# kazuotani14/iLQR

Measured on AMD Instinct MI355X. Metric: iLQR iterations/sec (batch x T timesteps/sec), acrobot T=500 batch=4096, higher is better.
Workload: dtype f64; 1 GPU; acrobot n=4 m=1 T=499 (500 knots), box-QP limits active, FD derivatives + backward/box-QP + 11-alpha search + accept, fixed work; batch_per_gpu=4096, global_batch=4096, T=499, parallelism=batch shards x1, one all_gather of costs

## Files before the change

ilqr_amd/csrc/backward_hex.hpp:

```cpp
#pragma once
#include "solve_tile.hpp"

namespace ilqr {

#ifndef ILQR_COMMIT_ROLLED
#define ILQR_COMMIT_ROLLED 1
#endif

constexpr int HT = 4;
#ifndef ILQR_HEX_SLOT_PAD
#define ILQR_HEX_SLOT_PAD 8
#endif
#ifndef ILQR_HEX_PAIR_PERM
#define ILQR_HEX_PAIR_PERM 1
#endif
#ifndef ILQR_HEX_CAND_T
#define ILQR_HEX_CAND_T 1
#endif
constexpr bool kHexCandT = ILQR_HEX_CAND_T != 0;

template <int NX, int NU, class real, int SLOTS_>
struct HexRing {
  static constexpr int US = Rec<NX, NU>::SIZE;
  static constexpr int PAIRS = (Rec<NX, NU>::SIZE + NU + 1) / 2;
  static constexpr int ROW = 2 * HT;
  static constexpr int PAD = ROW - 2 * TW;
  static constexpr int ELEMS = PAIRS * ROW + ILQR_HEX_SLOT_PAD;
  static constexpr int SLOTS = SLOTS_;
  static constexpr bool PERM = (ILQR_HEX_PAIR_PERM != 0) && NX == 4 && NU == 1;
  static constexpr int pos(int pair) { return PERM ? hex_pair_pos(pair) : pair; }
};

constexpr int kHexKnotsPerRound = 64 / HT;
constexpr int kHexSlots = 24;
constexpr int kHexLead = 7;
static_assert(kHexSlots > kHexLead + kHexKnotsPerRound - 1, "a round must not reach a slot the chain has not left");

template <class real, int NX, int NU>
struct HexPair {
  using RS = HexRing<NX, NU, real, kHexSlots>;
  alignas(16) real ring[RS::SLOTS * RS::ELEMS];
  int rounds_done;
  int consumer_at;
  int passes_started;
  unsigned long long pass_lanes;
};

template <class P>
struct HexGate {
  static constexpr bool kRing = true;
  P& sh;
  const int T, nrounds, N;
  int pass = -1, have = 0;
  int g_next = 0, slot_next = 0, slot_cur = 0;
  __device__ __forceinline__ HexGate(P& s, int T_) : sh(s), T(T_), nrounds((T_ + 1 + kHexKnotsPerRound - 1) / kHexKnotsPerRound), N(nrounds * kHexKnotsPerRound) {}
  __device__ __forceinline__ void begin_pass() {
    pass++;
    have = pass * N;
    g_next = pass * N;
    slot_next = g_next % P::RS::SLOTS;
    __hip_atomic_store(&sh.pass_lanes, __ballot(1), __ATOMIC_RELAXED, __HIP_MEMORY_SCOPE_WORKGROUP);
    __hip_atomic_store(&sh.passes_started, pass + 1, __ATOMIC_RELEASE, __HIP_MEMORY_SCOPE_WORKGROUP);
  }
  __device__ __forceinline__ int slot(int) const { return slot_cur; }
  __device__ __forceinline__ void wait(int) {
    const int G = g_next++;
    slot_cur = slot_next;
    slot_next = (slot_next + 1 == P::RS::SLOTS) ? 0 : slot_next + 1;
    __hip_atomic_store(&sh.consumer_at, G, __ATOMIC_RELAXED, __HIP_MEMORY_SCOPE_WORKGROUP);
    if (G < have) return;
    const int round = pass * nrounds + (G - pass * N) / kHexKnotsPerRound;
    while (__hip_atomic_load(&sh.rounds_done, __ATOMIC_ACQUIRE, __HIP_MEMORY_SCOPE_WORKGROUP) <= round) __builtin_amdgcn_s_sleep(1);
    have = pass * N + ((G - pass * N) / kHexKnotsPerRound + 1) * kHexKnotsPerRound;
  }
  __device__ __forceinline__ void finish() {
    __hip_atomic_store(&sh.consumer_at, 0x3fffffff, __ATOMIC_RELAXED, __HIP_MEMORY_SCOPE_WORKGROUP);
    __hip_atomic_store(&sh.passes_started, -1, __ATOMIC_RELEASE, __HIP_MEMORY_SCOPE_WORKGROUP);
  }
};

__device__ __forceinline__ int hex_first(unsigned long long bal, int t4) {
  return __builtin_ctzll(((bal >> t4) & 0x000F000F000F000Full) | 0x8000000000000000ull);
}
__device__ __forceinline__ void qp1_search_hex(QP1StateT<double>& q, int j, int t4, double step_j0, const double* __restrict__ lds_steps) {
  const double t_x1 = clamp_of(q.x + step_j0 * q.search, q.lo, q.hi);
  const double t_v1 = qp1_value(q, t_x1);
  const bool t_pass = !qp1_armijo_fails(q, t_v1, step_j0);
  const int pp = hex_first(__ballot(t_pass), t4);
  const bool success = pp < 52;
  const int jw = success ? (((pp >> 4) << 2) | (pp & 3)) : 0;
#ifdef ILQR_EXP_NO_STEP_LDS
  q.step = jw == 0 ? 1.0 : 0.6;
#else
  q.step = lds_steps[jw];
#endif
  q.x1 = clamp_of(q.x + q.step * q.search, q.lo, q.hi);
  q.v1 = qp1_value(q, q.x1);
  bool more = p_and(!success, !q.early);
  if (__builtin_expect(__ballot(more) == 0ull, 1)) return;
  {
    const bool stuck = p_and(j >= 1, t_x1 == q.x);
    const int qs = hex_first(__ballot(p_and(stuck, more)), t4);
    if (p_and(more, qs < 52)) {
      q.ls_failed = true;
      more = false;
    }
    if (__ballot(more) == 0ull) return;
  }
  for (int base = 16;; base += 16) {
    const int kn = base + j;
    const double my_step = lds_steps[kn < 104 ? kn : 103];
    const double my_x1 = qp1_trial(q, my_step);
    const double my_v1 = qp1_value(q, my_x1);
    const bool pass = !qp1_armijo_fails(q, my_v1, my_step);
    const bool stuck = p_or(my_step < kMinStep, my_x1 == q.x);
    const int qp = hex_first(__ballot(p_and(pass, more)), t4), qs = hex_first(__ballot(p_and(stuck, more)), t4);
    if (more) {
      if (qp < qs) {
        q.step = lds_steps[base + (((qp >> 4) << 2) | (qp & 3))];
        q.x1 = qp1_trial(q, q.step);
        q.v1 = qp1_value(q, q.x1);
        more = false;
      } else if (qs < 52) {
        q.ls_failed = true;
        more = false;
      }
    }
    if (__ballot(more) == 0ull) return;
  }
}

template <class RS>
__device__ __forceinline__ int hex_pos_rt(int pair) { return RS::PERM ? hex_pair_pos(pair) : pair; }

template <class real>
struct HexStep {
  typedef real pair_t __attribute__((ext_vector_type(2)));
  real F, cxx_rc, cxx_cr, fu_r, cx_r, cxu_r, cxu_c;
  pair_t tail, uw;
};

template <class M, class Gate, class RS>
__device__ __forceinline__ void backward_hex(const BatchViewT<typename M::real>& v, const M& model, const SolverParams& sp, int mode, int tile, int sub,
                                             int lane, const double* __restrict__ lds_steps, Gate& gate, const typename M::real* __restrict__ ring) {
  using real = typename M::real;
  using creal = double;
  static_assert(M::NX == 4 && M::NU == 1, "hex chain: nx = 4, nu = 1");
  using R = Rec<4, 1>;
  typedef real real2_t __attribute__((ext_vector_type(2)));
  const int r_ = lane >> 4, t_ = (lane >> 2) & 3, c_ = lane & 3, j16 = 4 * r_ + c_;
  const int t4 = 4 * t_;
  const int l = sub * HT + t_;
  const int b = tile * TW + l;
  if (b >= v.B) return;
  if (mode == 1 && v.status[b] != 0) return;
  const int T = v.T;
  double lambda = v.lambda[b], dlambda = v.dlambda[b];
  const real* __restrict__ ust = v.us + tidx(tile, 0, 0, l, T, 1);
  real* __restrict__ kt = v.kff + tidx(tile, 0, 0, l, T, 1);
  real* __restrict__ Kt = v.Kfb + tidx(tile, 0, 0, l, T, 4);
  typedef const __attribute__((address_space(3))) real lds_cd;
  typedef const __attribute__((address_space(3))) real2_t lds_cd2;
  const creal step_j0 = lds_steps[j16];
  auto mm = [](creal a, creal bb) __attribute__((always_inline)) { return __builtin_amdgcn_mfma_f64_4x4x4f64(a, bb, 0.0, 0, 0, 0); };

  auto load = [&](int t, HexStep<real>& d) __attribute__((always_inline)) {
    gate.wait(t);
    lds_cd* r = (lds_cd*)(ring + gate.slot(t) * RS::ELEMS + t_ * 2);
    auto pair = [&](int e) { return *(lds_cd2*)(r + RS::pos(e >> 1) * RS::ROW); };
    auto one = [&](int e) { return r[hex_pos_rt<RS>(e >> 1) * RS::ROW + (e & 1)]; };
    d.F = one(R::FX + r_ + 4 * c_);
    d.cxx_rc = one(R::CXX + r_ + 4 * c_);
    d.cxx_cr = one(R::CXX + c_ + 4 * r_);
    d.fu_r = one(R::FU + r_);
    d.cx_r = one(R::CX + r_);
    d.cxu_r = one(R::CXU + r_);
    d.cxu_c = one(R::CXU + c_);
    d.tail = pair(R::CU);
    d.uw = pair(RS::US);
  };

  int diverge = 0;
  bool done = false;
  double dV0 = 0, dV1 = 0, gacc = 0;
  auto one_pass = [&]() __attribute__((always_inline)) {
    gate.begin_pass();
    creal V, RVx, kprev;
    const creal lam_r = (creal)lambda;
    {
      gate.wait(T);
      lds_cd* r = (lds_cd*)(ring + gate.slot(T) * RS::ELEMS + t_ * 2);
      RVx = (creal)r[hex_pos_rt<RS>((R::CX + r_) >> 1) * RS::ROW + ((R::CX + r_) & 1)];
      V = (creal)r[hex_pos_rt<RS>((R::CXX + r_ + 4 * c_) >> 1) * RS::ROW + ((R::CXX + r_ + 4 * c_) & 1)];
    }
    kprev = (creal)kt[(unsigned)((T - 1) * TW)];
    __builtin_amdgcn_s_waitcnt(0x0F70);
    dV0 = dV1 = 0;
    diverge = 0;
    gacc = 0;
    real* __restrict__ Kt_i = Kt + (unsigned)(((T - 1) * 4 + c_) * TW);
    real* __restrict__ kt_i = kt + (unsigned)((T - 1) * TW);

    auto step = [&](int i, const HexStep<real>& raw, HexStep<real>& nxt) -> bool {
      const creal F = (creal)raw.F, Rfu = (creal)raw.fu_r;
      const creal cu = (creal)raw.tail.x, cuu = (creal)raw.tail.y, us = (creal)raw.uw.x, usw = (creal)raw.uw.y;
      const creal W = mm(V, F);
      const creal wv = mm(V, Rfu);
      const creal aQu = mm(Rfu, RVx);
      const creal aQx = mm(F, RVx);
      const creal Tm = mm(F, W);
      const creal Tt = mm(W, F);
      const creal aQuu = mm(Rfu, wv);
      const creal aQux_c = mm(Rfu, W);
      const creal aQux_r = mm(W, Rfu);
      const creal Qxx_rc = (creal)raw.cxx_rc + Tm, Qxx_cr = (creal)raw.cxx_cr + Tt;
      const creal Qx_r = (creal)raw.cx_r + aQx;
      const creal Qu = cu + aQu;
      const creal Qux_c = (creal)raw.cxu_c + aQux_c, Qux_r = (creal)raw.cxu_r + aQux_r;
      const creal Quu = cuu + aQuu, QuuF = (cuu + lam_r) + aQuu;
      const creal lo = (creal)model.u_min[0] - us, hi = (creal)model.u_max[0] - us;
      __builtin_amdgcn_sched_barrier(0);
      if (i >= 1) load(i - 1, nxt);
      __builtin_amdgcn_sched_barrier(0);
      creal x;
      int free0;
      creal minv;
      QP1StateT<creal> q1;
      qp1_begin<false>(QuuF, Qu, kprev, lo, hi, q1, false);
      qp1_search_hex(q1, j16, t4, step_j0, lds_steps);
      bool goes_on;
      bool ok = qp1_finish_ok(q1, x, free0, minv, goes_on);
      if (goes_on)
        ok = qp1_continue(
                 q1, [&](QP1StateT<creal>& qs) __attribute__((always_inline)) { qp1_search_hex(qs, j16, t4, step_j0, lds_steps); }, x, free0) >= 1;
      if (!ok) diverge = i;
      const creal k_scale = free0 ? -minv : creal(0);
      const creal K_r = k_scale * Qux_r, K_c = k_scale * Qux_c;
      creal d0 = 0, d1 = 0;
      {
        d0 += x * Qu;
        creal rq = 0;
        rq += (creal(0.5) * x) * Quu;
        d1 += rq * x;
      }
      creal T1_r, T1_c;
      {
        creal acc = 0;
        acc += K_r * Quu;
        T1_r = acc;
      }
      {
        creal acc = 0;
        acc += K_c * Quu;
        T1_c = acc;
      }
      creal Vxn_r, Vn_rc, Vn_cr;
      {
        creal t1 = 0, t2 = 0, t3 = 0;
        t1 += T1_r * x;
        t2 += K_r * Qu;
        t3 += Qux_r * x;
        Vxn_r = ((Qx_r + t1) + t2) + t3;
      }
      {
        creal u1 = 0, u2 = 0, u3 = 0;
        u1 += T1_r * K_c;
        u2 += K_r * Qux_c;
        u3 += Qux_r * K_c;
        Vn_rc = ((Qxx_rc + u1) + u2) + u3;
      }
      {
        creal u1 = 0, u2 = 0, u3 = 0;
        u1 += T1_c * K_r;
        u2 += K_c * Qux_r;
        u3 += Qux_c * K_r;
        Vn_cr = ((Qxx_cr + u1) + u2) + u3;
      }
      V = creal(0.5) * (Vn_rc + Vn_cr);
      RVx = Vxn_r;
      if (ok) {
        dV0 += (double)d0;
        dV1 += (double)d1;
        gacc += (double)(abs_of(x) * usw);
        kprev = (creal)(real)x;
        Kt_i[0] = (real)K_c;
        kt_i[0] = (real)x;
      }
      Kt_i -= 4 * TW;
      kt_i -= TW;
      return ok;
    };

    HexStep<real> A, Bd;
    int i = T - 1;
    load(i, A);
    while (true) {
      if (!step(i, A, Bd)) break;
      if (--i < 0) break;
      if (!step(i, Bd, A)) break;
      if (--i < 0) break;
    }
  };

  while (true) {
    one_pass();
    if (mode == 0) {
      done = (diverge == 0);
      break;
    }
    if (diverge != 0) {
      dlambda = fmax(dlambda * sp.lambda_factor, sp.lambda_factor);
      lambda = fmax(lambda * dlambda, sp.lambda_min);
      if (lambda > sp.lambda_max) break;
      continue;
    }
    done = true;
    break;
  }

  double acc = gacc;
  if (!done) {
    __builtin_amdgcn_fence(__ATOMIC_RELEASE, "workgroup");
    __builtin_amdgcn_s_waitcnt(0);
    acc = 0;
    for (int t0 = 0; t0 < T; t0 += 8) {
      real kv[8], uv[8];
#pragma unroll
      for (int jj = 0; jj < 8; jj++) {
        const int t = (t0 + jj < T) ? t0 + jj : T - 1;
        kv[jj] = kt[(size_t)t * TW];
        uv[jj] = ust[(size_t)t * TW];
      }
#pragma unroll
      for (int jj = 0; jj < 8; jj++) {
        const real mx = abs_of(kv[jj]) / (abs_of(uv[jj]) + 1);
        if (t0 + jj < T) acc += (double)mx;
      }
    }
  }
  const double gnorm = acc / T;
  if (j16 == 0) {
    v.dV[b] = dV0;
    v.dV[v.Bp + b] = dV1;
    v.diverge[b] = diverge;
    v.backpass_done[b] = done ? 1 : 0;
    v.gnorm[b] = gnorm;
    if (mode == 1) {
      v.lambda[b] = lambda;
      v.dlambda[b] = dlambda;
      if (!sp.fixed_work && gnorm < sp.tol_grad && lambda < 1e-5) {
        v.status[b] = 1;
        v.iters[b] += 1;
      }
    }
  }
}

template <class M, class MFD, class P>
__device__ __forceinline__ void sweep_backward_hex(const BatchViewT<typename M::real>& v, const M& model, const MFD& fdm, const SolverParams& sp, int mode,
                                                   int force, int tile, P* pairs, const double* __restrict__ lds_steps, int role) {
  using RS = typename P::RS;
  const int lane = threadIdx.x & 63;
  if (threadIdx.x < 4) {
    pairs[threadIdx.x].rounds_done = 0;
    pairs[threadIdx.x].consumer_at = 0;
    pairs[threadIdx.x].passes_started = 0;
  }
  __syncthreads();
  const int T = v.T;
  P& sh = pairs[role & 3];
  if (role < 4) {
    __builtin_amdgcn_s_setprio(3);
    HexGate<P> gate(sh, T);
    backward_hex<M, decltype(gate), RS>(v, model, sp, mode, tile, role, lane, lds_steps, gate, sh.ring);
    gate.finish();
    __builtin_amdgcn_s_setprio(0);
  } else {
    const int sub = role - 4;
    const int lp = lane & (HT - 1), ks = lane >> 2;
    const int l = sub * HT + lp;
    const int nrounds = (T + 1 + kHexKnotsPerRound - 1) / kHexKnotsPerRound, N = nrounds * kHexKnotsPerRound;
    for (int pass = 0;; pass++) {
      unsigned long long lanes = ~0ull;
      if (pass > 0) {
        int started;
        while ((started = __hip_atomic_load(&sh.passes_started, __ATOMIC_ACQUIRE, __HIP_MEMORY_SCOPE_WORKGROUP)) >= 0 && started <= pass)
          __builtin_amdgcn_s_sleep(8);
        if (started < 0) break;
        lanes = __hip_atomic_load(&sh.pass_lanes, __ATOMIC_RELAXED, __HIP_MEMORY_SCOPE_WORKGROUP);
      }
      const bool mine = (lanes >> (4 * lp)) & 1ull;
      for (int r = 0; r < nrounds; r++) {
        const int j0 = r * kHexKnotsPerRound, G0 = pass * N + j0;
        while (G0 > __hip_atomic_load(&sh.consumer_at, __ATOMIC_RELAXED, __HIP_MEMORY_SCOPE_WORKGROUP) + kHexLead) __builtin_amdgcn_s_sleep(4);
        const int started = __hip_atomic_load(&sh.passes_started, __ATOMIC_RELAXED, __HIP_MEMORY_SCOPE_WORKGROUP);
        if ((started < 0) | (started > pass + 1)) break;
        const int t = T - (j0 + ks);
        if (t >= 0 && (pass == 0 || mine))
          derivatives_of_knot<M, true, MFD, RS::PAD, RS::PERM>(v, model, fdm, force, nullptr, tile, t, l, sh.ring + ((G0 + ks) % RS::SLOTS) * RS::ELEMS + lp * 2, true);
        __builtin_amdgcn_s_waitcnt(0xC07F);
        if (lane == 0) __hip_atomic_store(&sh.rounds_done, pass * nrounds + r + 1, __ATOMIC_RELEASE, __HIP_MEMORY_SCOPE_WORKGROUP);
      }
    }
  }
}

template <class M, bool CANDT = false>
__device__ __forceinline__ void commit_tile_chunks(const BatchViewT<typename M::real>& v, const M& model, const int* commit_of_lane , int tile) {
  using real = typename M::real;
  constexpr int NX = M::NX, NU = M::NU;
  static_assert(!CANDT || (NX == 4 && NU == 1 && CT == 8 && CG == 4), "grouped candidates: nx = 4, nu = 1");
  const int T = v.T;
  const real dt = (real)v.dt;
  const int ntask = v.nch * TW;
  for (int task = threadIdx.x; task < ntask; task += blockDim.x) {
    const int l = task & (TW - 1), c = task >> 4;
    const int b = tile * TW + l;
    const int ci = (b < v.B) ? commit_of_lane[l] : -1;
    if (ci < 0) continue;
    const int ta = ci * v.ntiles + tile;
    real x[NX], uq[CT][NU];
    if constexpr (CANDT) {
      typedef real real4v __attribute__((ext_vector_type(4)));
      const real4v xv = *reinterpret_cast<const real4v*>(v.cand_x + cand_g_x(ta, c, l, v.nch, NX));
      x[0] = xv.x;
      x[1] = xv.y;
      x[2] = xv.z;
      x[3] = xv.w;
      const real4v u0 = *reinterpret_cast<const real4v*>(v.cand_u + cand_g_u(ta, 2 * c, l, T));
      const real4v u1 = *reinterpret_cast<const real4v*>(v.cand_u + cand_g_u(ta, 2 * c + 1, l, T));
      uq[0][0] = u0.x;
      uq[1][0] = u0.y;
      uq[2][0] = u0.z;
      uq[3][0] = u0.w;
      uq[4][0] = u1.x;
      uq[5][0] = u1.y;
      uq[6][0] = u1.z;
      uq[7][0] = u1.w;
    } else {
#pragma unroll
    for (int i = 0; i < NX; i++) x[i] = v.cand_x[tidx(ta, c, i, l, v.nch, NX)];
#pragma unroll
    for (int q = 0; q < CT; q++) {
      const int tq = (c * CT + q < T) ? c * CT + q : T - 1;
#pragma unroll
      for (int jj = 0; jj < NU; jj++) uq[q][jj] = v.cand_u[tidx(ta, tq, jj, l, T, NU)];
    }
    }
#if ILQR_COMMIT_ROLLED
#pragma unroll 1
    for (int q = 0; q < CT; q++) {
      const int t = c * CT + q;
      if (t > T) break;
#pragma unroll
      for (int i = 0; i < NX; i++) v.xs[tidx(tile, t, i, l, T + 1, NX)] = x[i];
      if (t < T) {
#pragma unroll
        for (int jj = 0; jj < NU; jj++) v.us[tidx(tile, t, jj, l, T, NU)] = uq[0][jj];
        if (q + 1 < CT) {
          real x1[NX];
          integrate_dynamics(model, x, uq[0], dt, x1);
#pragma unroll
          for (int i = 0; i < NX; i++) x[i] = x1[i];
        }
      }
#pragma unroll
      for (int qq = 0; qq + 1 < CT; qq++)
#pragma unroll
        for (int jj = 0; jj < NU; jj++) uq[qq][jj] = uq[qq + 1][jj];
    }
#else
#pragma unroll
    for (int q = 0; q < CT; q++) {
      const int t = c * CT + q;
      if (t <= T) {
#pragma unroll
        for (int i = 0; i < NX; i++) v.xs[tidx(tile, t, i, l, T + 1, NX)] = x[i];
        if (t < T) {
#pragma unroll
          for (int jj = 0; jj < NU; jj++) v.us[tidx(tile, t, jj, l, T, NU)] = uq[q][jj];
          if (q + 1 < CT) {
            real x1[NX];
            integrate_dynamics(model, x, uq[q], dt, x1);
#pragma unroll
            for (int i = 0; i < NX; i++) x[i] = x1[i];
          }
        }
      }
    }
#endif
  }
}

template <class M, class MFD>
__global__ __launch_bounds__(512) __attribute__((amdgpu_waves_per_eu(2, 2))) void k_solve_hex(BatchViewT<typename M::real> v, M model, MFD fdm, AlphaSet alphas,
                                                                                                 SolverParams sp, int n_iters, int force,
                                                                                                 int* __restrict__ commit_idx, int commit_pending,
                                                                                                 long long* __restrict__ phase_ticks) {
  using real = typename M::real;
  using P = HexPair<real, M::NX, M::NU>;
  __shared__ P pairs[4];
  __shared__ double steps[104];
  __shared__ double lds_cost[NALPHA * TW];
  __shared__ int tile_running;
  __shared__ int simd_count[4];
  __shared__ int lds_commit[TW];
  if (threadIdx.x < 4) simd_count[threadIdx.x] = 0;
  load_step_table(steps);
  const int wave = (int)(threadIdx.x >> 6);
  int role = wave;
  {
    const int simd = hw_simd_id();
    int slot = 0;
    if ((threadIdx.x & 63) == 0) slot = atomicAdd(&simd_count[simd], 1);
    slot = __shfl(slot, 0, 64);
    __syncthreads();
    if (simd_count[0] == 2 && simd_count[1] == 2 && simd_count[2] == 2 && simd_count[3] == 2) role = simd + 4 * slot;
  }
  const int rwave = (role < 3) ? role : 3;
  const int tile = blockIdx.x;
  constexpr int kShareReals = 4 * ((2 * M::NU + M::NU * M::NX + M::NX + 3) / 4) * TW;
  static_assert(kShareReals <= (int)(sizeof(pairs[0].ring) / sizeof(real)), "a pair's ring holds a wavefront's rollout rows");
  long long t_sweep = 0, t_roll = 0, t0 = 0;
#ifdef ILQR_HEX_SECTIONS
  long long t_sweep_last = 0;
#endif
  const bool timing = (phase_ticks != nullptr) & (threadIdx.x == 0);
  const long long c_begin = timing ? clock64() : 0, w_begin = timing ? wall_clock64() : 0;
  if (commit_pending) {
    commit_tile_chunks<M>(v, model, commit_idx + tile * TW, tile);
    phase_barrier();
  }
  int it = 0;
  for (; it < n_iters; it++) {
    if (timing) t0 = wall_clock64();
    sweep_backward_hex<M, MFD, P>(v, model, fdm, sp, 1, force, tile, pairs, steps, role);
    phase_barrier();
    if (timing) {
      const long long t1 = wall_clock64();
#ifdef ILQR_HEX_SECTIONS
      t_sweep_last = t1 - t0;
#endif
      t_sweep += t1 - t0;
      t0 = t1;
    }
    rollout_tile<M, true, true, kDeepPrefetch<M>, true, true, true, 1, kHexCandT>(v, model, alphas, NALPHA, v.cost_c, 1, sp, commit_idx, tile, lds_cost, it == n_iters - 1, rwave,
                                               pairs[role & 3].ring);
#ifdef ILQR_HEX_SECTIONS
#define ILQR_HEX_MARK(n)                                   \
    if (ILQR_HEX_SECTIONS == n && timing) {                \
      const long long t1 = wall_clock64();                 \
      t_sweep = t_sweep - t_sweep_last + (t1 - t0);        \
      t0 = t1;                                             \
    }
#else
#define ILQR_HEX_MARK(n)
#endif
    ILQR_HEX_MARK(1)
    if (threadIdx.x < TW) lds_commit[threadIdx.x] = commit_idx[tile * TW + threadIdx.x];
    if (threadIdx.x == 0) tile_running = 0;
    phase_barrier();
    ILQR_HEX_MARK(2)
    commit_tile_chunks<M, kHexCandT>(v, model, lds_commit, tile);
    ILQR_HEX_MARK(3)
    phase_barrier();
    if (timing) t_roll += wall_clock64() - t0;
    if (!sp.fixed_work) {
      const int b = tile * TW + (int)threadIdx.x;
      if (threadIdx.x < TW && b < v.B && v.status[b] == 0) tile_running = 1;
      __syncthreads();
      if (!tile_running) {
        it++;
        break;
      }
    }
  }
  if (timing) {
    phase_ticks[5 * tile + 0] += t_sweep;
    phase_ticks[5 * tile + 1] += t_roll;
    phase_ticks[5 * tile + 2] += it;
    phase_ticks[5 * tile + 3] += clock64() - c_begin;
    phase_ticks[5 * tile + 4] += wall_clock64() - w_begin;
  }
}

}
```

ilqr_amd/csrc/rollout.hpp:

```cpp
#pragma once
#include "layout.hpp"

namespace ilqr {

template <class View, class CostOf>
__device__ __forceinline__ void accept_one(const View& v, const SolverParams& sp, int b, CostOf cost_of,
                                           int* __restrict__ commit_idx, bool count_running = true) {
  if (b >= v.Bp) return;
  int commit = -1;
  if (b < v.B && v.status[b] == 0) {
    double lambda = v.lambda[b], dlambda = v.dlambda[b];
    const double cost_s = v.cost[b];
    bool fwd = false;
    double new_cost = 0, dcost = 0;
    int acc = -1;
    if (v.backpass_done[b]) {
      const double dV0 = v.dV[b], dV1 = v.dV[v.Bp + b];
      for (int a = 0; a < NALPHA; a++) {
        const double alpha = kAlpha[a];
        new_cost = cost_of(a);
        dcost = cost_s - new_cost;
        double expected;
        {
#pragma clang fp contract(off)
          expected = -alpha * (dV0 + alpha * dV1);
        }
        double z;
        if (expected > 0)
          z = dcost / expected;
        else
          z = (double)((0.0 < dcost) - (dcost < 0.0));
        if (z > sp.z_min) {
          fwd = true;
          acc = a;
          break;
        }
      }
    }
    int status = 0;
    if (fwd) {
      dlambda = fmin(dlambda / sp.lambda_factor, 1 / sp.lambda_factor);
      lambda = lambda * dlambda * (lambda > sp.lambda_min ? 1.0 : 0.0);
      v.cost[b] = new_cost;
      v.flg_change[b] = 1;
      commit = acc;
      if (!sp.fixed_work && dcost < sp.tol_fun) status = 2;
    } else {
      dlambda = fmax(dlambda * sp.lambda_factor, sp.lambda_factor);
      lambda = fmax(lambda * dlambda, sp.lambda_min);
      v.flg_change[b] = 0;
      if (!sp.fixed_work && lambda > sp.lambda_max) status = 3;
    }
    v.lambda[b] = lambda;
    v.dlambda[b] = dlambda;
    v.alpha_idx[b] = acc;
    const int it = v.iters[b] + 1;
    v.iters[b] = it;
    if (status == 0 && !sp.fixed_work && it >= sp.max_iter) status = 4;
    v.status[b] = status;
    if (status == 0 && count_running) atomicAdd(v.n_running, 1);
  }
  commit_idx[b] = commit;
}
template <class real>
__global__ void k_accept(BatchViewT<real> v, SolverParams sp, int* __restrict__ commit_idx) {
  const int b = blockIdx.x * blockDim.x + threadIdx.x;
  accept_one(v, sp, b, [&](int a) { return v.cost_c[(size_t)a * v.Bp + b]; }, commit_idx);
}

struct AlphaSet {
  double a[NALPHA];
};

#ifndef ILQR_ROLLOUT_UNCLAMPED_FETCH
#define ILQR_ROLLOUT_UNCLAMPED_FETCH 1
#endif
constexpr int kRolloutFetchSlack = 8;
constexpr size_t rollout_fetch_slack_elems(int nx, int nu) { return (size_t)kRolloutFetchSlack * nu * nx * TW; }
template <class M>
constexpr int kDeepPrefetch = (M::NU * M::NX + M::NX + 2 * M::NU <= 10) ? 8 : 4;

constexpr int CG = 4;
static_assert(CT % CG == 0, "a chunk of the commit is a whole number of control groups");
__host__ __device__ inline int cand_groups(int T) { return (T + CT + CG - 1) / CG; }
__host__ __device__ inline size_t cand_g_u(int ta, int grp, int l, int T) { return (((size_t)ta * cand_groups(T) + grp) * TW + l) * CG; }
__host__ __device__ inline size_t cand_g_x(int ta, int c, int l, int nch, int NX) { return (((size_t)ta * nch + c) * TW + l) * NX; }
template <class M, bool GAINS, bool CAND, int PD, bool ACCEPT, bool SHARE = false, bool NOFIX = false, int NG = 1, bool CANDT = false>
__device__ __forceinline__ void rollout_tile(const BatchViewT<typename M::real>& v, const M& model, const AlphaSet& alphas, int n_alpha,
                                             double* __restrict__ cost_out, int mode, const SolverParams& sp,
                                             int* __restrict__ commit_idx, int tile, double* lds_cost, bool count_running = true, int rwave = -1,
                                             typename M::real* share = nullptr) {
  using real = typename M::real;
  constexpr int NX = M::NX, NU = M::NU;
  static_assert(NG == 1 || (SHARE && GAINS && !ACCEPT), "several alpha groups per wavefront: the shared-row rollout of the wide tiles");
  static_assert(!CANDT || (CAND && SHARE && GAINS && NU == 1 && NX == 4 && PD % CG == 0), "grouped candidates: the matrix-core kernel's rollouts (nx = 4, nu = 1)");
  const int wave = (rwave >= 0) ? rwave : (int)(threadIdx.x >> 6);
  const int lane = threadIdx.x & 63;
  const int l = lane & (TW - 1);
  const int a_sub = lane >> 4;
  const int b = tile * TW + l;
  int a[NG];
  bool active[NG];
  bool any_active = false;
  const bool eligible = (b < v.B) && (mode != 1 || (v.status[b < v.B ? b : 0] == 0 && v.backpass_done[b < v.B ? b : 0]));
#pragma unroll
  for (int g = 0; g < NG; g++) {
    a[g] = (wave + g) * 4 + a_sub;
    active[g] = eligible && (a[g] < n_alpha);
    any_active = any_active || active[g];
  }
  const bool run = (SHARE && GAINS) ? (__ballot(any_active) != 0ull) : any_active;
  if (!ACCEPT && !run) return;
  if (run) {
  const int T = v.T;
  real alpha[NG];
#pragma unroll
  for (int g = 0; g < NG; g++) alpha[g] = (real)alphas.a[a[g] < NALPHA ? a[g] : NALPHA - 1];
  const real dt = (real)v.dt;

  real x[NG][NX];
#pragma unroll
  for (int i = 0; i < NX; i++) {
    const real x0i = v.x0[tidx(tile, 0, i, l, 1, NX)];
#pragma unroll
    for (int g = 0; g < NG; g++) x[g][i] = x0i;
  }
  double total[NG];
#pragma unroll
  for (int g = 0; g < NG; g++) total[g] = 0;

  struct StepIn {
    real u[NU], k[GAINS ? NU : 1], K[GAINS ? NU * NX : 1], xnom[GAINS ? NX : 1];
  };
  auto load_step = [&](int t, StepIn& d) __attribute__((always_inline)) {
    t = (t < T) ? t : T - 1;
#pragma unroll
    for (int j = 0; j < NU; j++) d.u[j] = v.us[tidx(tile, t, j, l, T, NU)];
    if (GAINS) {
#pragma unroll
      for (int j = 0; j < NU; j++) d.k[j] = v.kff[tidx(tile, t, j, l, T, NU)];
#pragma unroll
      for (int e = 0; e < NU * NX; e++) d.K[e] = v.Kfb[tidx(tile, t, e, l, T, NU * NX)];
#pragma unroll
      for (int i = 0; i < NX; i++) d.xnom[i] = v.xs[tidx(tile, t, i, l, T + 1, NX)];
    }
  };
  int ta_store[NG];
#pragma unroll
  for (int g = 0; g < NG; g++) ta_store[g] = ((SHARE && CAND && !active[g]) ? NALPHA : a[g]) * v.ntiles + tile;
  typedef real real4v __attribute__((ext_vector_type(4)));
  real pend[NG][CG - 1];
#pragma unroll
  for (int g = 0; g < NG; g++)
#pragma unroll
    for (int q = 0; q < CG - 1; q++) pend[g][q] = 0;
  auto store_group = [&](int g, int t, real last) __attribute__((always_inline)) {
    real4v w;
    w.x = pend[g][0];
    w.y = pend[g][1];
    w.z = pend[g][2];
    w.w = last;
    *reinterpret_cast<real4v*>(v.cand_u + cand_g_u(ta_store[g], t / CG, l, T)) = w;
  };
  auto emit_knot = [&](int g, int t, const real* xx, const real* uu, auto with_u, auto ph) __attribute__((always_inline)) {
    if (SHARE && !CAND && !active[g]) return;
    if constexpr (CANDT) {
      constexpr int p = decltype(ph)::value;
      if (with_u) {
        if constexpr (p == CG - 1)
          store_group(g, t, uu[0]);
        else
          pend[g][p] = uu[0];
      }
      if ((t & (CT - 1)) == 0) {
        real4v w;
        w.x = xx[0];
        w.y = xx[1];
        w.z = xx[2];
        w.w = xx[3];
        *reinterpret_cast<real4v*>(v.cand_x + cand_g_x(ta_store[g], t / CT, l, v.nch, NX)) = w;
      }
    } else if (CAND) {
      const int ta = ta_store[g];
      if (with_u) {
#pragma unroll
        for (int q = 0; q < NU; q++) v.cand_u[tidx(ta, t, q, l, T, NU)] = uu[q];
      }
      if ((t & (CT - 1)) == 0) {
#pragma unroll
        for (int i = 0; i < NX; i++) v.cand_x[tidx(ta, t / CT, i, l, v.nch, NX)] = xx[i];
      }
    } else {
#pragma unroll
      for (int i = 0; i < NX; i++) v.xs[tidx(tile, t, i, l, T + 1, NX)] = xx[i];
      if (with_u) {
#pragma unroll
        for (int q = 0; q < NU; q++) v.us[tidx(tile, t, q, l, T, NU)] = uu[q];
      }
    }
  };
  const WithTrigConsts<M> rmodel(model);
  auto do_step = [&](int t, const StepIn& d, auto ph) __attribute__((always_inline)) {
#pragma unroll
    for (int g = 0; g < NG; g++) {
      real u[NU];
#pragma unroll
      for (int j = 0; j < NU; j++) u[j] = d.u[j];
      if (GAINS) {
#pragma unroll
        for (int j = 0; j < NU; j++) {
          u[j] += d.k[j] * alpha[g];
          real acc = 0;
#pragma unroll
          for (int i = 0; i < NX; i++) acc += d.K[j + NU * i] * (x[g][i] - d.xnom[i]);
          u[j] += acc;
        }
      }
      if (!NOFIX && (sp.fixes & 1)) {
#pragma unroll
        for (int j = 0; j < NU; j++) u[j] = min_of(max_of(u[j], model.u_min[j]), model.u_max[j]);
      }
      emit_knot(g, t, x[g], u, std::true_type(), ph);
      total[g] += (double)model.cost(x[g], u);
      real x1[NX];
      integrate_dynamics(rmodel, x[g], u, dt, x1);
#pragma unroll
      for (int i = 0; i < NX; i++) x[g][i] = x1[i];
    }
  };
  if constexpr (SHARE && GAINS) {
    static_assert(PD % 2 == 0 || PD == 1, "static ring indices");
    static_assert((size_t)PD * NU * NX * TW <= rollout_fetch_slack_elems(NX, NU), "PD knots past the end");
    constexpr int NROWS = 2 * NU + NU * NX + NX;
    constexpr int NLD = (NROWS + 3) / 4;
    struct Raw {
      real r[NLD];
    };
    const real* rbase[NLD];
    unsigned rstride[NLD];
#pragma unroll
    for (int j = 0; j < NLD; j++) {
      const int row = (a_sub + 4 * j < NROWS) ? a_sub + 4 * j : NROWS - 1;
      if (row < NU) {
        rbase[j] = v.us + tidx(tile, 0, row, l, T, NU);
        rstride[j] = NU * TW;
      } else if (row < 2 * NU) {
        rbase[j] = v.kff + tidx(tile, 0, row - NU, l, T, NU);
        rstride[j] = NU * TW;
      } else if (row < 2 * NU + NU * NX) {
        rbase[j] = v.Kfb + tidx(tile, 0, row - 2 * NU, l, T, NU * NX);
        rstride[j] = NU * NX * TW;
      } else {
        rbase[j] = v.xs + tidx(tile, 0, row - 2 * NU - NU * NX, l, T + 1, NX);
        rstride[j] = NX * TW;
      }
    }
    auto fetch = [&](int tt, Raw& d) __attribute__((always_inline)) {
#if !ILQR_ROLLOUT_UNCLAMPED_FETCH
      tt = (tt < T) ? tt : T - 1;
#endif
#pragma unroll
      for (int j = 0; j < NLD; j++) d.r[j] = rbase[j][(size_t)tt * rstride[j]];
    };
    typedef real real2_t __attribute__((ext_vector_type(2)));
    constexpr int NPAIR = (NROWS + 1) / 2;
    real* const mine = share + (((a_sub >> 1) * TW + l) * 2 + (a_sub & 1));
    auto put = [&](const Raw& d) __attribute__((always_inline)) {
#pragma unroll
      for (int j = 0; j < NLD; j++) mine[4 * j * TW] = d.r[j];
    };
    const real2_t* const row0 = reinterpret_cast<const real2_t*>(share + 2 * l);
    auto get = [&](StepIn& d) __attribute__((always_inline)) {
      real rows[2 * NPAIR];
#pragma unroll
      for (int q = 0; q < NPAIR; q++) {
        const real2_t pr = row0[q * TW];
        rows[2 * q] = pr.x;
        rows[2 * q + 1] = pr.y;
      }
#pragma unroll
      for (int j = 0; j < NU; j++) d.u[j] = rows[j];
#pragma unroll
      for (int j = 0; j < NU; j++) d.k[j] = rows[NU + j];
#pragma unroll
      for (int e = 0; e < NU * NX; e++) d.K[e] = rows[2 * NU + e];
#pragma unroll
      for (int i = 0; i < NX; i++) d.xnom[i] = rows[2 * NU + NU * NX + i];
    };
    Raw ring[PD];
#pragma unroll
    for (int d = 0; d < PD; d++) fetch(d, ring[d]);
    StepIn cur, nxt;
    put(ring[0]);
    get(cur);
    auto one = [&](int s_, Raw& free_set, const Raw& next_set, auto ph) __attribute__((always_inline)) {
      put(next_set);
      get(nxt);
      fetch(s_ + PD, free_set);
      do_step(s_, cur, ph);
      cur = nxt;
    };
    int t = 0;
    for (; t + PD <= T; t += PD) {
      static_for<PD>([&](auto dc) __attribute__((always_inline)) {
        constexpr int d = decltype(dc)::value;
        one(t + d, ring[d], ring[(d + 1) % PD], std::integral_constant<int, d % CG>());
      });
    }
    static_for<PD>([&](auto dc) __attribute__((always_inline)) {
      constexpr int d = decltype(dc)::value;
      if (t + d < T) one(t + d, ring[d], ring[(d + 1) % PD], std::integral_constant<int, d % CG>());
    });
  } else {
  StepIn ring[PD];
#pragma unroll
  for (int d = 0; d < PD; d++) load_step(d, ring[d]);
  int t = 0;
  for (; t + PD <= T; t += PD) {
#pragma unroll
    for (int d = 0; d < PD; d++) {
      do_step(t + d, ring[d], std::integral_constant<int, 0>());
      load_step(t + d + PD, ring[d]);
    }
  }
  for (; t < T; t++) {
    StepIn cur;
    load_step(t, cur);
    do_step(t, cur, std::integral_constant<int, 0>());
  }
  }
#pragma unroll
  for (int g = 0; g < NG; g++) {
    {
      real uz[NU];
#pragma unroll
      for (int q = 0; q < NU; q++) uz[q] = 0;
      emit_knot(g, T, x[g], uz, std::false_type(), std::integral_constant<int, 0>());
      if constexpr (CANDT) {
        if (T % CG) store_group(g, T - 1, pend[g][CG - 2]);
      }
    }
    total[g] += (double)model.final_cost(x[g]);
    if (active[g]) {
      cost_out[(size_t)a[g] * v.Bp + b] = total[g];
      if (ACCEPT) lds_cost[a[g] * TW + l] = total[g];
    }
  }
  }
  if constexpr (ACCEPT) {
    __syncthreads();
    if (threadIdx.x < TW)
      accept_one(v, sp, tile * TW + (int)threadIdx.x, [&](int aa) { return lds_cost[aa * TW + threadIdx.x]; }, commit_idx, count_running);
  }
}

template <class M, bool GAINS, bool CAND, int PD = 4, bool ACCEPT = false>
__global__ __launch_bounds__(192) void k_rollout(BatchViewT<typename M::real> v, M model, AlphaSet alphas, int n_alpha,
                                                 double* __restrict__ cost_out, int mode, SolverParams sp,
                                                 int* __restrict__ commit_idx) {
  __shared__ double lds_cost[ACCEPT ? NALPHA * TW : 1];
  rollout_tile<M, GAINS, CAND, PD, ACCEPT>(v, model, alphas, n_alpha, cost_out, mode, sp, commit_idx, (int)blockIdx.x, lds_cost);
}

template <class M, bool CANDT = false>
__device__ __forceinline__ void candidate_knot(const BatchViewT<typename M::real>& v, const M& model, int a, int tile, int t, int l,
                                               typename M::real* x, typename M::real* u) {
  using real = typename M::real;
  constexpr int NX = M::NX, NU = M::NU;
  const int T = v.T, ta = a * v.ntiles + tile, c = t / CT, off = t - c * CT;
#pragma unroll
  for (int i = 0; i < NX; i++) x[i] = CANDT ? v.cand_x[cand_g_x(ta, c, l, v.nch, NX) + i] : v.cand_x[tidx(ta, c, i, l, v.nch, NX)];
  real uq[CT][NU];
#pragma unroll
  for (int q = 0; q < CT; q++) {
    const int tq = (c * CT + q < T) ? c * CT + q : T - 1;
#pragma unroll
    for (int j = 0; j < NU; j++) uq[q][j] = CANDT ? v.cand_u[cand_g_u(ta, tq / CG, l, T) + tq % CG] : v.cand_u[tidx(ta, tq, j, l, T, NU)];
  }
#pragma unroll
  for (int j = 0; j < NU; j++) u[j] = 0.0;
#pragma unroll
  for (int q = 0; q < CT; q++) {
    if (q < off) {
      real x1[NX];
      integrate_dynamics(model, x, uq[q], (real)v.dt, x1);
#pragma unroll
      for (int i = 0; i < NX; i++) x[i] = x1[i];
    }
    if (q == off && t < T) {
#pragma unroll
      for (int j = 0; j < NU; j++) u[j] = uq[q][j];
    }
  }
}

template <class M, bool CANDT = false>
__global__ void k_unpack_cand(BatchViewT<typename M::real> v, M model, int a, double* __restrict__ xs, double* __restrict__ us) {
  using real = typename M::real;
  constexpr int NX = M::NX, NU = M::NU;
  const int T = v.T;
  const size_t n = (size_t)v.B * (T + 1);
  for (size_t i = (size_t)blockIdx.x * blockDim.x + threadIdx.x; i < n; i += (size_t)gridDim.x * blockDim.x) {
    const int t = (int)(i % (T + 1));
    const int b = (int)(i / (T + 1));
    real x[NX], u[NU];
    candidate_knot<M, CANDT>(v, model, a, b / TW, t, b % TW, x, u);
    if (xs)
      for (int e = 0; e < NX; e++) xs[((size_t)b * (T + 1) + t) * NX + e] = (double)x[e];
    if (us && t < T)
      for (int e = 0; e < NU; e++) us[((size_t)b * T + t) * NU + e] = (double)u[e];
  }
}

}
```

Before: 4.321 billion trajectory-timesteps/s.

## Add a feeder wavefront that streams rollout rows into a shared LDS ring

The fourth wavefront (role 3) becomes a producer during the rollout. It loads the gains, controls and nominal states from global memory in rounds of eight knots into a three-round LDS ring and signals progress through workgroup-scope atomics. The three rollout wavefronts then read their step rows from that ring instead of each issuing its own prefetch and sharing through its pair's ring. The aim is to take global-load latency and per-wave fetch work off the consumer waves. In exchange it adds spin-wait handshakes with s_sleep and a single ring all consumers depend on, so one slow wave can stall the others.

```diff
diff --git a/ilqr_amd/csrc/backward_hex.hpp b/ilqr_amd/csrc/backward_hex.hpp
--- a/ilqr_amd/csrc/backward_hex.hpp
+++ b/ilqr_amd/csrc/backward_hex.hpp
@@ -519,8 +519,10 @@
   }
   const int rwave = (role < 3) ? role : 3;
   const int tile = blockIdx.x;
-  constexpr int kShareReals = 4 * ((2 * M::NU + M::NU * M::NX + M::NX + 3) / 4) * TW;
-  static_assert(kShareReals <= (int)(sizeof(pairs[0].ring) / sizeof(real)), "a pair's ring holds a wavefront's rollout rows");
+  static_assert(kFeedRingReals<M> <= (int)(sizeof(pairs[0].ring) / sizeof(real)), "a pair's ring holds the rollouts' feed ring");
+  static_assert(kFeedRingReals<M> == kFeedRounds * kFeedKnots * 10 * TW, "three rounds of eight steps of ten rows: 30 720 bytes in double");
+  __shared__ int feed_ctl[kFeedCtl];
+  if (threadIdx.x < kFeedCtl) feed_ctl[threadIdx.x] = 0;
   long long t_sweep = 0, t_roll = 0, t0 = 0;
 #ifdef ILQR_HEX_SECTIONS
   long long t_sweep_last = 0;
@@ -544,8 +546,8 @@
       t_sweep += t1 - t0;
       t0 = t1;
     }
-    rollout_tile<M, true, true, kDeepPrefetch<M>, true, true, true, 1, kHexCandT>(v, model, alphas, NALPHA, v.cost_c, 1, sp, commit_idx, tile, lds_cost, it == n_iters - 1, rwave,
-                                               pairs[role & 3].ring);
+    rollout_tile<M, true, true, kDeepPrefetch<M>, true, true, true, 1, kHexCandT, true>(v, model, alphas, NALPHA, v.cost_c, 1, sp, commit_idx, tile, lds_cost, it == n_iters - 1, rwave,
+                                               pairs[3].ring, feed_ctl, role == 3);
 #ifdef ILQR_HEX_SECTIONS
 #define ILQR_HEX_MARK(n)                                   \
     if (ILQR_HEX_SECTIONS == n && timing) {                \
@@ -559,6 +561,7 @@
     ILQR_HEX_MARK(1)
     if (threadIdx.x < TW) lds_commit[threadIdx.x] = commit_idx[tile * TW + threadIdx.x];
     if (threadIdx.x == 0) tile_running = 0;
+    if (threadIdx.x < kFeedCtl) feed_ctl[threadIdx.x] = 0;
     phase_barrier();
     ILQR_HEX_MARK(2)
     commit_tile_chunks<M, kHexCandT>(v, model, lds_commit, tile);
diff --git a/ilqr_amd/csrc/rollout.hpp b/ilqr_amd/csrc/rollout.hpp
--- a/ilqr_amd/csrc/rollout.hpp
+++ b/ilqr_amd/csrc/rollout.hpp
@@ -80,18 +80,90 @@
 template <class M>
 constexpr int kDeepPrefetch = (M::NU * M::NX + M::NX + 2 * M::NU <= 10) ? 8 : 4;
 
+template <class M>
+__device__ __forceinline__ void rollout_row(const BatchViewT<typename M::real>& v, int tile, int l, int row, const typename M::real*& base, unsigned& stride) {
+  constexpr int NX = M::NX, NU = M::NU;
+  const int T = v.T;
+  if (row < NU) {
+    base = v.us + tidx(tile, 0, row, l, T, NU);
+    stride = NU * TW;
+  } else if (row < 2 * NU) {
+    base = v.kff + tidx(tile, 0, row - NU, l, T, NU);
+    stride = NU * TW;
+  } else if (row < 2 * NU + NU * NX) {
+    base = v.Kfb + tidx(tile, 0, row - 2 * NU, l, T, NU * NX);
+    stride = NU * NX * TW;
+  } else {
+    base = v.xs + tidx(tile, 0, row - 2 * NU - NU * NX, l, T + 1, NX);
+    stride = NX * TW;
+  }
+}
+
+constexpr int kFeedKnots = 8;
+constexpr int kFeedRounds = 3;
+constexpr int kFeedCtl = 4;
+static_assert(kFeedKnots <= kRolloutFetchSlack, "a round past the end stays inside the slack");
+template <class M>
+constexpr int kFeedStepReals = ((2 * M::NU + M::NU * M::NX + M::NX + 1) / 2) * 2 * TW;
+template <class M>
+constexpr int kFeedRingReals = kFeedRounds * kFeedKnots * kFeedStepReals<M>;
+__host__ __device__ inline int feed_rounds(int T) { return T / kFeedKnots + 1; }
+__host__ __device__ inline int feed_consumers(int n_alpha) { return n_alpha >= 9 ? 3 : (n_alpha + 3) / 4; }
+
+template <class M>
+__device__ __forceinline__ void rollout_feed_tile(const BatchViewT<typename M::real>& v, int n_alpha, int mode, int tile, typename M::real* ring, int* ctl) {
+  using real = typename M::real;
+  constexpr int NX = M::NX, NU = M::NU;
+  constexpr int NROWS = 2 * NU + NU * NX + NX, NLD = (NROWS + 3) / 4, R = kFeedKnots;
+  static_assert((size_t)R * NU * NX * TW <= rollout_fetch_slack_elems(NX, NU), "a round of knots past the end");
+  const int lane = threadIdx.x & 63, l = lane & (TW - 1), a_sub = lane >> 4;
+  const int b = tile * TW + l;
+  const bool eligible = (b < v.B) && (mode != 1 || (v.status[b < v.B ? b : 0] == 0 && v.backpass_done[b < v.B ? b : 0]));
+  const int nc = feed_consumers(n_alpha);
+  if (__ballot(eligible) == 0ull || nc == 0) return;
+  const int nrounds = feed_rounds(v.T);
+  const real* rbase[NLD];
+  unsigned rstride[NLD];
+#pragma unroll
+  for (int j = 0; j < NLD; j++) rollout_row<M>(v, tile, l, (a_sub + 4 * j < NROWS) ? a_sub + 4 * j : NROWS - 1, rbase[j], rstride[j]);
+  real* const mine = ring + (((a_sub >> 1) * TW + l) * 2 + (a_sub & 1));
+  int slot = 0;
+  for (int r = 0; r < nrounds; r++) {
+    real val[R][NLD];
+#pragma unroll
+    for (int d = 0; d < R; d++)
+#pragma unroll
+      for (int j = 0; j < NLD; j++)
+        if (a_sub + 4 * j < NROWS) val[d][j] = rbase[j][(size_t)(r * R + d) * rstride[j]];
+    if (r >= kFeedRounds) {
+      for (int w = 0; w < nc; w++)
+        while (__hip_atomic_load(&ctl[1 + w], __ATOMIC_ACQUIRE, __HIP_MEMORY_SCOPE_WORKGROUP) < (r - kFeedRounds + 1) * R) __builtin_amdgcn_s_sleep(4);
+    }
+    real* const dst = mine + slot * (R * kFeedStepReals<M>);
+#pragma unroll
+    for (int d = 0; d < R; d++)
+#pragma unroll
+      for (int j = 0; j < NLD; j++)
+        if (a_sub + 4 * j < NROWS) dst[d * kFeedStepReals<M> + 4 * j * TW] = val[d][j];
+    slot = (slot + 1 == kFeedRounds) ? 0 : slot + 1;
+    __builtin_amdgcn_s_waitcnt(0xC07F);
+    if (lane == 0) __hip_atomic_store(&ctl[0], (r + 1) * R, __ATOMIC_RELEASE, __HIP_MEMORY_SCOPE_WORKGROUP);
+  }
+}
+
 constexpr int CG = 4;
 static_assert(CT % CG == 0, "a chunk of the commit is a whole number of control groups");
 __host__ __device__ inline int cand_groups(int T) { return (T + CT + CG - 1) / CG; }
 __host__ __device__ inline size_t cand_g_u(int ta, int grp, int l, int T) { return (((size_t)ta * cand_groups(T) + grp) * TW + l) * CG; }
 __host__ __device__ inline size_t cand_g_x(int ta, int c, int l, int nch, int NX) { return (((size_t)ta * nch + c) * TW + l) * NX; }
-template <class M, bool GAINS, bool CAND, int PD, bool ACCEPT, bool SHARE = false, bool NOFIX = false, int NG = 1, bool CANDT = false>
+template <class M, bool GAINS, bool CAND, int PD, bool ACCEPT, bool SHARE = false, bool NOFIX = false, int NG = 1, bool CANDT = false, bool FEED = false>
 __device__ __forceinline__ void rollout_tile(const BatchViewT<typename M::real>& v, const M& model, const AlphaSet& alphas, int n_alpha,
                                              double* __restrict__ cost_out, int mode, const SolverParams& sp,
                                              int* __restrict__ commit_idx, int tile, double* lds_cost, bool count_running = true, int rwave = -1,
-                                             typename M::real* share = nullptr) {
+                                             typename M::real* share = nullptr, int* feed_ctl = nullptr, bool feeder = false) {
   using real = typename M::real;
   constexpr int NX = M::NX, NU = M::NU;
+  static_assert(!FEED || (SHARE && GAINS && ACCEPT && NG == 1 && (!CANDT || kFeedKnots % CG == 0)), "fed rows: the matrix-core kernel's rollouts");
   static_assert(NG == 1 || (SHARE && GAINS && !ACCEPT), "several alpha groups per wavefront: the shared-row rollout of the wide tiles");
   static_assert(!CANDT || (CAND && SHARE && GAINS && NU == 1 && NX == 4 && PD % CG == 0), "grouped candidates: the matrix-core kernel's rollouts (nx = 4, nu = 1)");
   const int wave = (rwave >= 0) ? rwave : (int)(threadIdx.x >> 6);
@@ -111,6 +183,9 @@
   }
   const bool run = (SHARE && GAINS) ? (__ballot(any_active) != 0ull) : any_active;
   if (!ACCEPT && !run) return;
+  if constexpr (FEED) {
+    if (feeder) rollout_feed_tile<M>(v, n_alpha, mode, tile, share, feed_ctl);
+  }
   if (run) {
   const int T = v.T;
   real alpha[NG];
@@ -270,11 +345,11 @@
       for (int j = 0; j < NLD; j++) mine[4 * j * TW] = d.r[j];
     };
     const real2_t* const row0 = reinterpret_cast<const real2_t*>(share + 2 * l);
-    auto get = [&](StepIn& d) __attribute__((always_inline)) {
+    auto get_at = [&](StepIn& d, const real2_t* rowp) __attribute__((always_inline)) {
       real rows[2 * NPAIR];
 #pragma unroll
       for (int q = 0; q < NPAIR; q++) {
-        const real2_t pr = row0[q * TW];
+        const real2_t pr = rowp[q * TW];
         rows[2 * q] = pr.x;
         rows[2 * q + 1] = pr.y;
       }
@@ -287,6 +362,44 @@
 #pragma unroll
       for (int i = 0; i < NX; i++) d.xnom[i] = rows[2 * NU + NU * NX + i];
     };
+    auto get = [&](StepIn& d) __attribute__((always_inline)) { get_at(d, row0); };
+    if constexpr (FEED) {
+      constexpr int R = kFeedKnots, STEP2 = kFeedStepReals<M> / 2;
+      static_assert(2 * NPAIR * TW == kFeedStepReals<M>, "the feeder's step image is the one `get` reads");
+      int* const my_at = feed_ctl + 1 + wave;
+      int slot = 0;
+      const real2_t* rp = row0;
+      auto wait_step = [&](int s) __attribute__((always_inline)) {
+        while (__builtin_expect(__builtin_amdgcn_readfirstlane(__hip_atomic_load(&feed_ctl[0], __ATOMIC_ACQUIRE, __HIP_MEMORY_SCOPE_WORKGROUP)) <= s, 0))
+          __builtin_amdgcn_s_sleep(1);
+      };
+      StepIn cur, nxt;
+      wait_step(0);
+      get_at(cur, rp);
+      auto one = [&](int s_, auto dc, auto ph) __attribute__((always_inline)) {
+        constexpr int d = decltype(dc)::value;
+        if constexpr (d == R - 1) {
+          __hip_atomic_store(my_at, s_ + 1, __ATOMIC_RELEASE, __HIP_MEMORY_SCOPE_WORKGROUP);
+          slot = (slot + 1 == kFeedRounds) ? 0 : slot + 1;
+          rp = row0 + slot * (R * STEP2);
+          wait_step(s_ + 1);
+          get_at(nxt, rp);
+        } else {
+          get_at(nxt, rp + (d + 1) * STEP2);
+        }
+        do_step(s_, cur, ph);
+        cur = nxt;
+      };
+      int t = 0;
+      for (; t + R <= T; t += R) {
+        static_for<R>([&](auto dc) __attribute__((always_inline)) { one(t + decltype(dc)::value, dc, std::integral_constant<int, decltype(dc)::value % CG>()); });
+      }
+      static_for<R - 1>([&](auto dc) __attribute__((always_inline)) {
+        constexpr int d = decltype(dc)::value;
+        if (t + d < T) one(t + d, dc, std::integral_constant<int, d % CG>());
+      });
+      __hip_atomic_store(my_at, feed_rounds(T) * R, __ATOMIC_RELEASE, __HIP_MEMORY_SCOPE_WORKGROUP);
+    } else {
     Raw ring[PD];
 #pragma unroll
     for (int d = 0; d < PD; d++) fetch(d, ring[d]);
@@ -311,6 +424,7 @@
       constexpr int d = decltype(dc)::value;
       if (t + d < T) one(t + d, ring[d], ring[(d + 1) % PD], std::integral_constant<int, d % CG>());
     });
+    }
   } else {
   StepIn ring[PD];
 #pragma unroll
```

Result: no change. 4.360 billion trajectory-timesteps/s, median of 6 (+0.9%).
